# seqsense/pcgol

Measured on AMD Instinct MI355X. Metric: Mpoints/sec ICP iter (corr+reduce) + kNN queries/sec, 1M-pt cloud, higher is better.
Workload: dtype f32

## Files before the change

pcgol_amd/csrc/icp.hip:

```cpp
#include <string.h>

#include <array>
#include <chrono>
#include <condition_variable>
#include <mutex>
#include <string>
#include <thread>

#include <vector>

#include "knn_grid.h"
#include "knn_xwalk.h"
#include "icp_step_plan.h"
#include "strict_terms.h"
#include "gicp_terms.h"

namespace pcgx {

constexpr int kIcpBlock = kKnnBlock;

__device__ __forceinline__ double wave_sum_f64(double v) {
#pragma unroll
  for (int o = 32; o > 0; o >>= 1) v += __shfl_down(v, o);
  return v;
}

__device__ __forceinline__ void accumulate_terms(double *acc, float x0, float y0, float z0, const float4 &bp,
                                                 const IcpKernelParams &kp) {
  const float x1 = bp.x, y1 = bp.y, z1 = bp.z;
  const float w = eval_weight_fn(kp.weight_fn, kp.weight_a, bp.w);
  acc[S_VALUE] += (double)(w * bp.w);
  acc[S_G0 + 0] += (double)(w * (x0 - x1));
  acc[S_G0 + 1] += (double)(w * (y0 - y1));
  acc[S_G0 + 2] += (double)(w * (z0 - z1));
// ... 639 lines not shown
  uint32_t *d_dropped = nullptr;
  int gicp_grid = 1;
  int n_sums() const { return plane ? (int)P_COUNT : (int)S_COUNT; }
  int grid = 1;
  IcpKernelParams kp;
  int32_t max_iteration = 20;
};

static pcgx_status settle(pcgx_icp_session *s, hipStream_t st);
static int icp_knob(const char *name, int def, int lo, int hi);

static IcpKernelParams make_kernel_params(const pcgx_icp_params *p) {
  IcpKernelParams kp;
  memset(&kp, 0, sizeof kp);
  kp.max_dist_sq = p->max_dist * p->max_dist;
  kp.min_dist_sq = p->min_dist_sq;
  kp.min_pairs = p->min_pairs == 0 ? 6 : p->min_pairs;
  kp.upd = resolve_updater(p->weight, p->threshold, p->max_iteration);
  kp.gn = resolve_gauss_newton(p->threshold, 0.0f, p->max_iteration);
  kp.weight_fn = p->weight_fn;
  kp.weight_a = p->weight_fn_param;
  return kp;
}

static int icp_grid(int64_t nt, const TreeView &tv) {
  int64_t blocks = (nt + kIcpBlock - 1) / kIcpBlock;
  int64_t cap = (int64_t)ctx().num_cu * walk_blocks_per_cu(tv) * walk_oversubscribe();
  if (blocks > cap) blocks = cap;
  if (blocks >= 8) blocks &= ~(int64_t)7;
  if (blocks < 1) blocks = 1;
  return (int)blocks;
}

__global__ void icp_reset_kernel(IcpState *__restrict__ state) {
  if (threadIdx.x != 0 || blockIdx.x != 0) return;
  IcpState h;
  memset(&h, 0, sizeof h);
  const Mat4 id = mat4_translate(0.0f, 0.0f, 0.0f);
  for (int i = 0; i < 16; i++) h.trans[i] = id.m[i];
  *state = h;
}

static pcgx_status general_prepare(pcgx_icp_session *s, hipStream_t st) {
  if (s->general_ready) return PCGX_OK;
  const size_t n1 = (size_t)(s->nt ? s->nt : 1);
  PCGX_HIP_TRY(hipMemsetAsync(s->d_match, 0xFF, n1 * sizeof(float4), st));
  PCGX_HIP_TRY(hipMemsetAsync(s->d_match_cert, 0, n1 * sizeof(float), st));
  PCGX_HIP_TRY(hipMemsetAsync(s->d_first_leaf, 0, n1 * sizeof(uint32_t), st));
  PCGX_HIP_TRY(hipMemsetAsync(s->d_walk_count, 0, (size_t)s->grid * sizeof(uint32_t), st));
  s->general_ready = true;
  return PCGX_OK;
}

static pcgx_status reset_state(pcgx_icp_session *s, hipStream_t st) {
  hipLaunchKernelGGL(icp_reset_kernel, dim3(1), dim3(64), 0, st, s->d_state);
  PCGX_HIP_TRY(hipGetLastError());
  s->host_iter = 0;
  if (s->spec_pending) {
    s->spec_pending = false;
    if (s->d_walk_count) PCGX_HIP_TRY(hipMemsetAsync(s->d_walk_count, 0, (size_t)s->grid * sizeof(uint32_t), st));
    PCGX_TRY(strict_reset(s->strict_buf, st));
  }
  if (s->shard_failed || s->steps_sharded > 0) {
    PCGX_TRY(strict_reset(s->strict_buf, st));
    s->shard_failed = false;
    s->steps_sharded = 0;
  }
  return PCGX_OK;
}

extern "C" pcgx_status pcgx_icp_session_reset(pcgx_icp_session *s, void *stream) {
  PCGX_API_LOCK();
  if (!s) return fail(PCGX_E_INVALID, "pcgx_icp_session_reset: NULL session");
  s->touch(pick_stream(stream));
  return reset_state(s, pick_stream(stream));
}

extern "C" pcgx_status pcgx_icp_session_set_pose(pcgx_icp_session *s, const float trans16[16],
                                                 int32_t iter, void *stream) {
  PCGX_API_LOCK();
  if (!s || !trans16 || iter < 0) return fail(PCGX_E_INVALID, "pcgx_icp_session_set_pose: bad argument");
  hipStream_t st = pick_stream(stream);
  s->touch(st);
  PCGX_TRY(settle(s, st));
  IcpState h;
  memset(&h, 0, sizeof h);
  memcpy(h.trans, trans16, sizeof h.trans);
  h.iter = iter;
  s->host_iter = 0;
  PCGX_HIP_TRY(hipMemcpyAsync(s->d_state, &h, sizeof h, hipMemcpyHostToDevice, st));
  PCGX_HIP_TRY(hipStreamSynchronize(st));
  return PCGX_OK;
}

extern "C" pcgx_status pcgx_icp_session_read_sums(pcgx_icp_session *s, double sums10[10], void *stream) {
// ... 1136 lines not shown
```

pcgol_amd/csrc/pcgx_internal.h:

```cpp
#pragma once
#include <hip/hip_runtime.h>
#include <stdint.h>
#include <stdio.h>
#include <stdlib.h>

#include <atomic>
#include <memory>
#include <mutex>
#include <string>
#include <utility>
#include <vector>

#include "../../include/pcgx.h"
#include "pcgx_math.h"

namespace pcgx {

template <class T>
struct DefaultInitAlloc : std::allocator<T> {
  template <class U>
  struct rebind {
    using other = DefaultInitAlloc<U>;
  };
  template <class U>
// ... 220 lines not shown
  UpdaterParams upd;
  GaussNewtonParams gn;
  int32_t weight_fn;
  float weight_a;
};


#if defined(__HIPCC__)
constexpr unsigned int kTicketGroups = 32u, kTicketStride = 32u;
static_assert((1u + kTicketGroups) * kTicketStride * 4u <= kTicketBytes, "the context's ticket words");
__device__ __forceinline__ bool last_workgroup_ticket(unsigned int *tickets) {
  const unsigned int g = blockIdx.x & (kTicketGroups - 1u), groups = min(gridDim.x, kTicketGroups);
  const unsigned int members = (gridDim.x - g + kTicketGroups - 1u) / kTicketGroups;
  unsigned int *mine = tickets + kTicketStride * (1u + g);
  if (atomicAdd(mine, 1u) != members - 1u) return false;
  __hip_atomic_store(mine, 0u, __ATOMIC_RELAXED, __HIP_MEMORY_SCOPE_AGENT);
  if (atomicAdd(tickets, 1u) != groups - 1u) return false;
  __hip_atomic_store(tickets, 0u, __ATOMIC_RELAXED, __HIP_MEMORY_SCOPE_AGENT);
  return true;
}

__device__ __forceinline__ uint32_t wave_incl_scan_u32(uint32_t v) {
#define PCGX_DPP_ADD(CTRL, MASK) v += (uint32_t)__builtin_amdgcn_update_dpp(0, (int)v, CTRL, MASK, 0xf, (MASK) == 0xf)
  PCGX_DPP_ADD(0x111, 0xf);
  PCGX_DPP_ADD(0x112, 0xf);
  PCGX_DPP_ADD(0x114, 0xf);
  PCGX_DPP_ADD(0x118, 0xf);
  PCGX_DPP_ADD(0x142, 0xa);
  PCGX_DPP_ADD(0x143, 0xc);
#undef PCGX_DPP_ADD
  return v;
}
__device__ __forceinline__ void icp_update_step(IcpState *__restrict__ state, const double *__restrict__ sums10,
                                                const IcpKernelParams &kp) {
  state->num_iteration += 1;
  const int64_t npairs = (int64_t)sums10[S_PAIRS];
  if (npairs < (int64_t)kp.min_pairs) {
    state->ev.num_pairs = npairs;
    state->status = PCGX_E_NOT_ENOUGH_PAIRS;
    state->done = 1;
    return;
  }
  Evaluated ev;
  finish_evaluate(sums10, ev);
  state->ev = ev;
  Mat4 t;
  for (int i = 0; i < 16; i++) t.m[i] = state->trans[i];
  int32_t it = state->iter;
  const bool converged = gradient_descent_update(kp.upd, it, ev.gradient, t);
  for (int i = 0; i < 16; i++) state->trans[i] = t.m[i];
  state->iter = it;
  if (converged) state->done = 1;
}

#endif

struct StrictBuffers;
struct StrictWork;
struct CertifiedTerms;
pcgx_status strict_create(int64_t nt, const float *tx, const float *ty, const float *tz, const uint32_t *pos_of,
                          StrictBuffers **out, hipStream_t st);
void strict_destroy(StrictBuffers *b);
const StrictWork *strict_work(StrictBuffers *b, const IcpKernelParams &kp);
pcgx_status strict_enqueue(StrictBuffers *b, const float4 *match, const uint32_t *pos_of, IcpState *state,
                           double *sums10, const IcpKernelParams &kp, bool fuse_update, bool have_tile_sums, bool first_iter,
                           hipStream_t st, const struct CertifiedTerms *certify = nullptr);
pcgx_status strict_read_debug(StrictBuffers *b, unsigned long long out[64], hipStream_t st);
pcgx_status strict_check_enqueue(const float *d_xyz, int64_t nt, int64_t nt_pad, const float4 *match, const uint32_t *pos_of,
                                 IcpState *state, const IcpKernelParams &kp, float *d_terms, unsigned long long *d_valid,
                                 double *d_sums, bool fuse_update, hipStream_t st);
pcgx_status strict_enqueue_sharded(StrictBuffers *b, const float4 *match, const uint32_t *pos_of, IcpState *state,
                                   double *sums10, const IcpKernelParams &kp, pcgx_comm *c, int rank, int world,
                                   bool local_failed, hipStream_t st);
struct RingView {
  unsigned long long *words = nullptr;
  unsigned long long *host = nullptr;
  unsigned long long *const *tab = nullptr;
  unsigned long long *mine = nullptr;
  int32_t words_per_rank = 0, rank = 0, world = 1;
  uint32_t epoch = 0;
  int32_t kind = 0;
  long long guess_ticks = 0;
};
pcgx_status strict_enqueue_ring(StrictBuffers *b, const float4 *match, const uint32_t *pos_of, IcpState *state, double *sums10,
                                const IcpKernelParams &kp, const RingView &ring, bool local_failed, bool first_iter, hipStream_t st);
void ring_abort_from_host(const RingView &ring, uint32_t reason);
pcgx_status strict_reset(StrictBuffers *b, hipStream_t st);
bool small_fit_eligible(const TreeView &tv, int64_t nt, bool many_ties);
size_t small_fit_sync_bytes();
size_t small_fit_terms_bytes(int64_t nt);
int small_fit_max_iters();
bool small_fit_wants_order(int64_t nt);
pcgx_status small_fit_prepare(const float *d_target_aos, int64_t nt, const float box_lo[3], const float box_hi[3], int32_t *d_perm, float *d_xyz,
                               uint32_t *d_pos_of, IcpState *state, void *terms, void *sync, hipStream_t st);
pcgx_status small_fit_enqueue(const TreeView &tv, const float *tx, const float *ty, const float *tz, int64_t nt, IcpState *state,
                              const IcpKernelParams &kp, void *terms, unsigned long long *valid, double *sums10, void *sync,
                              uint32_t launch_no, int iters, const int32_t *perm, hipStream_t st, volatile uint32_t *mailbox = nullptr,
                              uint32_t mailbox_seq = 0u);
bool comm_ring_step(pcgx_comm *c, int32_t step, RingView *out);
void comm_ring_new_fit(pcgx_comm *c);
int comm_ring_kind(pcgx_comm *c);
void comm_attach_local_ring(pcgx_comm *c, unsigned long long *block, int32_t words_per_rank);
}

struct pcgx_kdtree {
  int64_t n = 0;
  int32_t depth = 0;
  float4 *d_nodes = nullptr;
  uint32_t *d_dir = nullptr;
  uint32_t *d_inv = nullptr;
  int32_t dir_bits = 0;
  float dir_lo[3] = {0, 0, 0}, dir_scale[3] = {0, 0, 0};
  float bbox_lo[3] = {0, 0, 0}, bbox_hi[3] = {0, 0, 0};
  bool has_nan = false;
  bool many_ties = false;
  pcgx::RawVector<int32_t> inorder;
  pcgx::RawVector<float> points;
  struct XNode {
    int32_t id, c0, c1, dim;
  };
// ... 35 lines not shown
```

pcgol_amd/csrc/strict.hip:

```cpp
#include <stddef.h>

#include "knn_grid.h"
#include "strict_terms.h"

namespace pcgx {

__device__ __forceinline__ int lane_next(int v, int edge) { return __builtin_amdgcn_update_dpp(edge, v, 0x130, 0xf, 0xf, false); }
__device__ __forceinline__ int lane_prev(int v, int edge) { return __builtin_amdgcn_update_dpp(edge, v, 0x138, 0xf, 0xf, false); }
__device__ __forceinline__ double wave_excl_scan_f64(double v, int lane) {
  double inc = v;
  inc += dpp_f64<0x111, 0xf>(0.0, inc);
  inc += dpp_f64<0x112, 0xf>(0.0, inc);
  inc += dpp_f64<0x114, 0xf>(0.0, inc);
  inc += dpp_f64<0x118, 0xf>(0.0, inc);
  inc += dpp_f64<0x142, 0xa>(0.0, inc);
  inc += dpp_f64<0x143, 0xc>(0.0, inc);
  (void)lane;
  return dpp_f64<0x138, 0xf>(0.0, inc);
}
__device__ __forceinline__ uint32_t wave_all_umin(uint32_t v) {
#define PCGX_DPP_U32(CTRL, MASK) (uint32_t) __builtin_amdgcn_update_dpp(-1, (int)v, CTRL, MASK, 0xf, false)
  v = umin(v, PCGX_DPP_U32(0x111, 0xf));
  v = umin(v, PCGX_DPP_U32(0x112, 0xf));
  v = umin(v, PCGX_DPP_U32(0x114, 0xf));
// ... 260 lines not shown
                                             ChainRange &cr, double &tile_err) {
  g = f2u((float)(base + pre));
  const float e = u2f(plain_chain_q(q, g));
  const double err = ((double)e - (double)u2f(g)) - lsum;
  const double epre = wave_excl_scan_f64(err, lane);
  tile_err = lane_f64(epre, 63) + lane_f64(err, 63);
  const uint32_t g2 = f2u((float)(base + pre + epre));
  const int32_t moved = (int32_t)g2 - (int32_t)g;
  if (__ballot(moved > 2 || moved < -2) != 0ull) g = g2;
  cr = guess_chain_q(q, g);
}
__device__ __forceinline__ void tile_guesses_pair(const LdsQuads &q, double base, double lsum, double pre, int lane, uint32_t &g,
                                                  ChainRange &cr, ChainRange &crb, double &tile_err) {
  g = f2u((float)(base + pre));
  const float e = u2f(plain_chain_q(q, g));
  const double err = ((double)e - (double)u2f(g)) - lsum;
  const double epre = wave_excl_scan_f64(err, lane);
  tile_err = lane_f64(epre, 63) + lane_f64(err, 63);
  const uint32_t g2 = f2u((float)(base + pre + epre));
  const int32_t moved = (int32_t)g2 - (int32_t)g;
  if (__ballot(moved > 2 || moved < -2) != 0ull) g = g2;
  guess_chain_pair_q(q, g, cr, crb);
}

constexpr int kExactTiles = 1;
constexpr uint32_t kPlainMargin = 512u;
constexpr uint32_t kMaybeMargin = 1u << 17;

constexpr int kSumBlock = 512;
constexpr int kSumWaves = kSumBlock / 64;
enum { JOB_CROSSING = 1, JOB_NOWINDOW = 2 };

constexpr long long kExchangeTicks = 200000;
__device__ __forceinline__ void certified_search(const CertifiedTerms &C, const TermSrc &S, const IcpState *state, const StrictWork &W,
                                                 int64_t tile, const uint16_t *list, int nl, float4 *terms ,
                                                 int *np_more) {
  TermSrc S0 = S;
  S0.project = false;
  for (int j = threadIdx.x; j < nl; j += kSumBlock) {
    const int q = list[j];
    const int64_t c = tile * kTile + q;
    float x = W.xyz_caller[3 * c], y = W.xyz_caller[3 * c + 1], z = W.xyz_caller[3 * c + 2];
    float ub = __builtin_inff();
    if (S.project) {
      float px, py, pz;
      mat4_transform(S.m, x, y, z, px, py, pz);
      x = px; y = py; z = pz;
      const float4 pm = C.match_caller[c];
      const float dx = pm.x - x, dy = pm.y - y, dz = pm.z - z;
      const float dm = (dx * dx + dy * dy) + dz * dz;
      if (pm.w >= 0.0f && dm == dm) ub = dm;
    }
    float4 best = make_float4(0.0f, 0.0f, 0.0f, __int_as_float(-1));
    float best_d = C.max_dist_sq;
    GridVerdict v = grid_nearest(C.grid, x, y, z, C.max_dist_sq, ub, best, best_d);
    if (C.test_force_grid_walk && c % C.test_force_grid_walk == 0) v = GRID_WALK;
    if (v == GRID_WALK) {
      if (atomicCAS(&const_cast<IcpState *>(state)->done, 0, 2) == 0) atomicAdd(&W.dbg[47], 1ull << 32);
      continue;
    }
    const bool found = __float_as_int(best.w) >= 0;
    const float cert = (v == GRID_FOUND && found) ? C.grid.cert[__float_as_uint(best.w)] : 0.0f;
    const uint32_t pos = C.pos_of[c];
    C.match[pos] = make_float4(best.x, best.y, best.z, found ? best_d : -1.0f);
    C.match_cert[pos] = cert;
    C.match_caller[c] = make_float4(best.x, best.y, best.z, found ? cert : -1.0f);
    if (found) {
      float t[kStrictRows];
      (void)pair_terms(S0, x, y, z, make_float4(best.x, best.y, best.z, best_d), t);
      const int l = q / kLeaf, vq = (q % kLeaf) / 4, cc = q % 4;
#pragma unroll
      for (int k = 0; k < kStrictRows; k++) reinterpret_cast<float *>(&terms[k * (kTile / 4) + tile_quad(l, vq)])[cc] = t[k];
      atomicAdd(np_more, 1);
    }
  }
}

template <bool kExchange, bool kSharded = false, bool kCertify = false>
__global__ __launch_bounds__(kSumBlock) __attribute__((amdgpu_waves_per_eu(4, 4))) void strict_sum_kernel(
    const float4 *__restrict__ match, const uint32_t *__restrict__ pos_of, const IcpState *__restrict__ state, StrictWork W,
    CertifiedTerms C = CertifiedTerms()) {
  __shared__ float4 s_terms[kStrictRows][kTile / 4];
  __shared__ int s_np[kSumWaves];
  __shared__ double s_tot[16];
  __shared__ uint16_t s_list[kCertify ? kTile : 1];
  __shared__ int s_nlist, s_np_more;
  static_assert(!kSharded || kExchange, "the ring form rides on the exchange");
  static_assert(!kCertify || (kExchange && !kSharded), "the certified terms: one GPU, with the exchange");
  const int done = state->done;
  const int lane = threadIdx.x & 63, wave = threadIdx.x >> 6;
  const int64_t tile = blockIdx.x;
  const int NR = W.nrows;
  const long long t_0 = trace_clock(W);
  long long t_x0 = 0;
  double P0 = (!kExchange && wave < NR) ? tile_prefix(W.tile_sum, W.ntiles, wave, tile, lane) : 0.0;
  {
    const TermSrc S = make_term_src(match, pos_of, state, W);
    const int l = threadIdx.x >> 3, v = threadIdx.x & 7;
    float4 bp[4];
    float tx[4], ty[4], tz[4];
    const int64_t i0 = tile * kTile + (int64_t)l * kLeaf + 4 * v;
    load_quad(S, i0, bp, tx, ty, tz);
    if (kCertify) {
      if (threadIdx.x == 0) s_nlist = s_np_more = 0;
      __syncthreads();
    }
    float t[4][kStrictRows];
    int np = 0;
#pragma unroll
    for (int c = 0; c < 4; c++) {
      if (kCertify) {
        float x = tx[c], y = ty[c], z = tz[c];
        if (S.project) mat4_transform(S.m, tx[c], ty[c], tz[c], x, y, z);
        const float dx = bp[c].x - x, dy = bp[c].y - y, dz = bp[c].z - z;
        const float dm = (dx * dx + dy * dy) + dz * dz;
        bool kept = S.project && bp[c].w >= 0.0f && dm < bp[c].w && dm < C.max_dist_sq;
        if ((C.test_force_walk && (i0 + c) % C.test_force_walk == 0) || (C.test_force_grid_walk && (i0 + c) % C.test_force_grid_walk == 0))
          kept = false;
        if (!kept && i0 + c < W.nt) {
          s_list[atomicAdd(&s_nlist, 1)] = (uint16_t)(l * kLeaf + 4 * v + c);
          bp[c].w = -1.0f;
        }
      }
      np += pair_terms(S, tx[c], ty[c], tz[c], bp[c], t[c]) ? 1 : 0;
    }
#pragma unroll
    for (int k = 0; k < kStrictRows; k++) s_terms[k][tile_quad(l, v)] = make_float4(t[0][k], t[1][k], t[2][k], t[3][k]);
#pragma unroll
    for (int o = 32; o > 0; o >>= 1) np += __shfl_xor(np, o);
    if (lane == 0) s_np[wave] = np;
  }
  __syncthreads();
  if (done) return;
  if (kCertify) {
    const int nl = s_nlist;
    if (nl > 0) {
      certified_search(C, make_term_src(match, pos_of, state, W), state, W, tile, s_list, nl, &s_terms[0][0], &s_np_more);
      __syncthreads();
    }
    if (threadIdx.x == 0) {
      if (tile == 0) atomicAdd(&W.dbg[47], 1ull);
      if (nl > 0) atomicAdd(&W.dbg[59], (unsigned long long)nl);
    }
  }
  if (threadIdx.x == 0) {
    int np = kCertify ? s_np_more : 0;
    for (int w = 0; w < kSumWaves; w++) np += s_np[w];
    W.tile_pairs[tile] = (uint32_t)np;
  }
  static_assert(kStrictRows <= 2 * kSumWaves, "a wave has at most two rows");
  double lsum_kept[2] = {0.0, 0.0}, pre_kept[2] = {0.0, 0.0};
  if (kExchange) {
#pragma unroll
    for (int pass = 0; pass < 2; pass++) {
      const int row = wave + pass * kSumWaves;
      if (row >= NR) break;
      const LdsQuads q{s_terms[row], lane};
      double lsum = 0.0;
#pragma unroll
      for (int v = 0; v < kLeaf / 4; v++) {
        const float4 a = q(v);
        lsum += (double)a.x; lsum += (double)a.y; lsum += (double)a.z; lsum += (double)a.w;
      }
      const double pre = wave_excl_scan_f64(lsum, lane);
      lsum_kept[pass] = lsum;
      pre_kept[pass] = pre;
      if (lane == 63) s_tot[row] = pre + lsum;
    }
    __syncthreads();
    t_x0 = trace_clock(W);
    if (wave == 0) {
      if (lane < NR) {
        const double v = s_tot[lane];
        __hip_atomic_store(&W.tile_pub[(int64_t)lane * W.ntiles_pad + tile], v, __ATOMIC_RELAXED, __HIP_MEMORY_SCOPE_AGENT);
        W.tile_sum[(int64_t)lane * W.ntiles + tile] = v;
      }
      asm volatile("s_waitcnt vmcnt(0)" ::: "memory");
      const int64_t g_mine = tile >> 5, n_groups = (W.ntiles + 31) >> 5;
      if (lane == 0) {
// ... 152 lines not shown
      }
      T.s = par_expand(S, E, key);
      if (lane == 0) W.recs[row * W.ntiles + tile] = T;
      maybe_E = (m_lo < kMaybeMargin || m_hi > 0x7fffffu - kMaybeMargin) ? (int32_t)E : -1;
      if (maybe_E < 0) continue;
    }
    unsigned slot = 0xffffffffu;
    const unsigned shard = (unsigned)((tile + 7 * row) % kAuxShards), per_shard = (unsigned)W.naux / kAuxShards;
    if (lane == 0) {
      const unsigned k = atomicAdd(&W.aux_count[shard * 32], 1u);
      slot = k < per_shard ? shard * per_shard + k : 0xffffffffu;
    }
    slot = (unsigned)rfl((int)slot);
    if (slot == 0xffffffffu) {
      if (maybe_E < 0) {
        T.key = -1;
        T.cons = 0;
        if (lane == 0) W.recs[row * W.ntiles + tile] = T;
      }
      continue;
    }
    if (lane == 0) {
      JobDesc *J = W.jobs + slot;
      J->row = row;
      J->tile = tile;
      J->pad = maybe_E >= 0 ? (1 | (maybe_E << 8)) : 0;
    }
    float4 *dst = W.aux_terms + (size_t)slot * (kTile / 4);
    int lane_here = lane;
    asm volatile("" : "+v"(lane_here));
#pragma unroll
    for (int v = 0; v < kLeaf / 4; v++) dst[v * kLanes + lane_here] = s_terms[row][v * kLanes + lane_here];
  }
  if (threadIdx.x == 0 && (W.selfcheck & 2)) {
    W.stamps[tile * 16 + 0] = (unsigned long long)t_0;
    W.stamps[tile * 16 + 1] = (unsigned long long)t_1;
    W.stamps[tile * 16 + 2] = (unsigned long long)t_x0;
    W.stamps[tile * 16 + 5] = (unsigned long long)trace_clock(W);
  }
}

constexpr int kJobBlock = 256;
constexpr int kJobRoles = 3;
template <bool kRegs>
__device__ __forceinline__ uint32_t resolve_staged(uint32_t s, int kind, int32_t key, const LeafAux &A, int lane,
                                               const float4 *lds, const float *t, int &serial_out, int &tried_out,
                                               int &applied_out);
__global__ __launch_bounds__(kJobBlock) void strict_job_kernel(const IcpState *__restrict__ state, StrictWork W) {
  __shared__ float4 s_t[kTile / 4];
  __shared__ float4 s_lin[kTile / 4];
  __shared__ int32_t s_S[12][kLanes];
  __shared__ uint32_t s_g[kLanes];
  __shared__ int32_t s_lk[kLanes];
  __shared__ int32_t s_hdr[5];
  __shared__ uint32_t s_ctab[4][kCandInner];
  __shared__ int s_cdone, s_pieces;
  const unsigned per_shard = (unsigned)W.naux / kAuxShards;
  const int lane = threadIdx.x & 63, part = threadIdx.x >> 6;
  const int role = (int)(blockIdx.x % kJobRoles);
  const unsigned jb = blockIdx.x / kJobRoles;
  const unsigned shard = jb % kAuxShards, slot = shard * per_shard + jb / kAuxShards;
  const JobDesc *J = W.jobs + slot;
  const float4 *src4 = W.aux_terms + (size_t)slot * (kTile / 4);
  static_assert(kTile / 4 == 2 * kJobBlock, "two quads of the tile per thread");
  const bool early = jb / kAuxShards < 6;
  float4 q0 = make_float4(0.0f, 0.0f, 0.0f, 0.0f), q1 = q0;
  int row = 0, pad = 0;
  int64_t tile = 0;
  if (early) {
    q0 = src4[threadIdx.x];
// ... 544 lines not shown
struct ChainMail {
  int req;
  int ack;
  uint32_t s_in, s_out;
};

template <bool kCheck, bool kSpec = false>
__global__ __launch_bounds__(kChainBlock) void strict_chain_kernel(const float4 *__restrict__ match,
                                                                  const uint32_t *__restrict__ pos_of,
                                                                  IcpState *__restrict__ state, StrictWork W,
                                                                  double *__restrict__ sums10, IcpKernelParams kp,
                                                                  int fuse_update) {
  __shared__ RecArray s_rec;
  __shared__ RecArray s_pre;
  __shared__ RecArray s_suf;
  __shared__ int16_t s_tail[kChainTiles];
  __shared__ int16_t s_head[kChainTiles];
  __shared__ int16_t s_auxlist[kChainTiles];
  __shared__ int16_t s_auxord[kChainTiles];
  __shared__ int32_t s_count[kChainSegs], s_auxcnt[kChainSegs];
  __shared__ uint32_t s_auxmask[kChainSegs][2];
  __shared__ int s_sufok[kChainSegs];
  __shared__ int s_pre_cnt[2];
  __shared__ int s_progress;
  __shared__ ChainMail s_mail[kChainSegs];
  __shared__ uint32_t s_tab[kTabSlots][kCand];
  __shared__ int s_tab_ord[kTabSlots];
  __shared__ float4 s_tile[kTile / 4];
  __shared__ unsigned long long s_np;
  __shared__ int s_np_ok;
  __shared__ uint32_t s_stat[8];
  __shared__ unsigned long long s_wk[8];
  __shared__ unsigned long long s_stat_ticks[2];
  const int done = state->done;
  const int row = (int)(blockIdx.x % (unsigned)W.nrows), my_chunk = (int)(blockIdx.x / (unsigned)W.nrows);
  const int lane = threadIdx.x & 63, wave = rfl((int)(threadIdx.x >> 6));
  const bool walker = wave == kWalker;
  const bool last_chunk = my_chunk == W.nchunks - 1;
  auto term_src = [&]() { return make_term_src(match, pos_of, state, W); };
  uint32_t s = W.start_bits ? (uint32_t)rfl((int)W.start_bits[row]) : f2u(0.0f);
  int ring_rc = 0;
  auto row_start = [&]() -> uint32_t {
    if (!W.ring || W.rank == 0) return W.start_bits ? (uint32_t)rfl((int)W.start_bits[row]) : f2u(0.0f);
    const RingLayout RL{W.world};
    uint32_t v = 0u;
    ring_rc = ring_wait(W, RL.start(row), v, kRingWalkTicks);
    if (ring_rc == 2 && lane == 0) ring_raise_abort(W, 0x100u | (uint32_t)row);
    return (uint32_t)rfl((int)v);
  };
  uint32_t n_run = 0, n_runfail = 0, n_recfail = 0, n_tab_nw = 0, n_tab_cross = 0;
  uint32_t n_mail = 0;
  asm volatile("" : "+v"(n_run), "+v"(n_runfail), "+v"(n_recfail), "+v"(n_tab_nw), "+v"(n_tab_cross), "+v"(n_mail));
  unsigned long long ticks_scan = 0, ticks_walk = 0;
  const long long t_enter = trace_clock(W);
  const unsigned long long c_enter = (W.selfcheck & 2) ? (unsigned long long)__builtin_readcyclecounter() : 0ull;
  {
    const int64_t chunk = (int64_t)my_chunk * kChainTiles;
    const long long t_a = stat_clock(W);
    if (threadIdx.x < kChainSegs) {
      s_sufok[threadIdx.x] = 0;
      s_mail[threadIdx.x].req = 0;
      s_mail[threadIdx.x].ack = 0;
    }
    if (threadIdx.x < kTabSlots) s_tab_ord[threadIdx.x] = 0;
    if (threadIdx.x == 0) {
      s_progress = 0;
      s_pre_cnt[0] = s_pre_cnt[1] = 0;
      s_np_ok = 0;
    }
    if (threadIdx.x < 8) s_wk[threadIdx.x] = 0ull;
    TileRec R;
    R.key = -2;
    R.in = R.out = 0u;
    R.cons = 0;
    R.s = summary_identity();
    bool head = true, tail = true, valid = false;
    {
      const int64_t tile = chunk + threadIdx.x;
      valid = tile < W.ntiles;
      if (valid) R = W.recs[row * W.ntiles + tile];
      if ((W.selfcheck & 2) && last_chunk && walker) {
        const unsigned long long tt = clock_after((uint32_t)R.key);
        if (lane == 0) s_wk[4] = tt;
      }
      rec_put(s_rec, threadIdx.x, R);
      const int32_t key_prev = lane_prev(R.key, R.key), key_next = lane_next(R.key, R.key);
      const int alone = stands_alone(R) ? 1 : 0, alone_prev = lane_prev(alone, 0), alone_next = lane_next(alone, 0);
      head = lane == 0 || R.key < 0 || R.key != key_prev || alone || alone_prev;
      tail = lane == 63 || R.key < 0 || R.key != key_next || alone || alone_next;
      const unsigned long long tails = __ballot(tail && valid);
      if (tail && valid) {
        const unsigned long long below = tails & ((1ull << lane) - 1ull);
        const int idx = wave * 64 + __popcll(below);
        s_tail[idx] = (int16_t)threadIdx.x;
        s_head[idx] = (int16_t)(wave * 64 + (below ? 64 - __builtin_clzll(below) : 0));
      }
      if (lane == 0) s_count[wave] = __popcll(tails);
      const unsigned long long aux = __ballot(valid && (R.cons >> 8) != 0);
      if (lane == 0) {
        s_auxcnt[wave] = __popcll(aux);
        s_auxmask[wave][0] = (uint32_t)aux;
        s_auxmask[wave][1] = (uint32_t)(aux >> 32);
      }
// ... 784 lines not shown
      return;
    }
    if (row == 0 && lane == 0) __hip_atomic_store(&sums10[S_PAIRS], (double)pairs, __ATOMIC_RELAXED, __HIP_MEMORY_SCOPE_AGENT);
  } else if (row == 0 && walker && lane == 0) {
    while (lds_get(&s_np_ok) == 0) __builtin_amdgcn_s_sleep(1);
    if (!W.hop_out) __hip_atomic_store(&sums10[S_PAIRS], (double)s_np, __ATOMIC_RELAXED, __HIP_MEMORY_SCOPE_AGENT);
  }
  if (walker) {
    unsigned ticket = 0u;
    if (lane == 0) {
      const int slot = row == 0 ? S_VALUE : (row <= 6 ? S_G0 + row - 1 : (row == 7 ? S_DIST_RMS : S_WEIGHT));
      if (W.hop_out) W.hop_out[row] = (double)s;
      else __hip_atomic_store(&sums10[slot], (double)u2f(s), __ATOMIC_RELAXED, __HIP_MEMORY_SCOPE_AGENT);
      if (W.hop_out) __threadfence();
      else asm volatile("s_waitcnt vmcnt(0)" ::: "memory");
      ticket = atomicAdd(W.done_rows, 1u);
    }
    ticket = (unsigned)rfl((int)ticket);
    if (ticket == (unsigned)W.nrows - 1u) {
      static_assert(kAuxShards == kLanes, "a shard's counter per lane");
      W.aux_count[lane * 32] = 0u;
      if (W.exchange)
        for (int64_t k = lane, n = (W.ntiles + 31) / 32, m = n + (n + 31) / 32; k < m; k += kLanes) W.tile_arrived[32 * k] = 0u;
      if (lane == 0) *W.done_rows = 0u;
      if (!W.hop_out && lane == 0) {
        double sums[S_COUNT];
        for (int k = 0; k < S_COUNT; k++) sums[k] = __hip_atomic_load(&sums10[k], __ATOMIC_RELAXED, __HIP_MEMORY_SCOPE_AGENT);
        const unsigned long long np = (unsigned long long)sums[S_PAIRS];
        if (W.nrows < kStrictRows) {
          sums[S_WEIGHT] = (double)(np < (1ull << 24) ? np : (1ull << 24));
          sums10[S_WEIGHT] = sums[S_WEIGHT];
        }
        const long long t_u0 = trace_clock(W);
        if (fuse_update) icp_update_step(state, sums, kp);
        if (W.selfcheck & 2) {
          __threadfence();
          W.stamps[kStrictRows * 16 + 14] = (unsigned long long)t_u0;
          W.stamps[kStrictRows * 16 + 15] = (unsigned long long)trace_clock(W);
        }
      }
    }
  }
}

struct StrictBuffers {
  StrictWork w;
  void *block = nullptr;
  double *shard = nullptr;
  int shard_world = 0;
  bool shard_ring = false;
  void *counters = nullptr;
  size_t counters_bytes = 0, arrived_bytes = 0;
};

pcgx_status strict_create(int64_t nt, const float *tx, const float *ty, const float *tz, const uint32_t *pos_of,
                          StrictBuffers **out, hipStream_t st) {
  StrictBuffers *b = new StrictBuffers();
  StrictWork &W = b->w;
  W.nt = nt;
  W.raw_terms = nullptr;
  W.row_base = W.err_base = nullptr;
  W.start_bits = nullptr;
  W.hop_out = nullptr;
  W.first_exact = 1;
  W.ring = nullptr;
  W.ring_words = 0;
  W.ring_tab = nullptr;
// ... 347 lines not shown
    ProfScope prof(PCGX_PROF_STRICT_SUM, st);
    hipLaunchKernelGGL((strict_sum_kernel<true, true>), dim3((unsigned)W.ntiles), dim3(kSumBlock), 0, st, match, pos_of,
                       (const IcpState *)state, W);
  }
  if (ring.world > 1)
    hipLaunchKernelGGL(strict_ring_err_kernel, dim3(kStrictRows + (ring.rank > 0 ? 1 : 0)), dim3(64), 0, st, (const IcpState *)state, W);
  if (ring.rank > 0) {
    W.row_base = W.ring_base;
    W.err_base = W.ring_base + 16;
  }
  {
    ProfScope prof(PCGX_PROF_STRICT_JOB, st);
    if (first_iter && W.naux > 0 && W.ntiles >= kRepairMinTiles && repair_enabled())
      hipLaunchKernelGGL(strict_repair_kernel, dim3((unsigned)(W.nrows * ((W.ntiles + kRepairBlock - 1) / kRepairBlock))), dim3(kRepairBlock), 0,
                         st, match, pos_of, (const IcpState *)state, W);
    if (W.naux > 0)
      hipLaunchKernelGGL(strict_job_kernel, dim3((unsigned)kJobRoles * (unsigned)W.naux), dim3(kJobBlock), 0, st, (const IcpState *)state, W);
  }
  {
    ProfScope prof(PCGX_PROF_STRICT_CHAIN, st);
    launch_chain(W, match, pos_of, state, sums10, kp, 1, true, st);
  }
  PCGX_HIP_TRY(hipGetLastError());
  return PCGX_OK;
}

pcgx_status strict_reset(StrictBuffers *b, hipStream_t st) {
  if (!b) return PCGX_OK;
  PCGX_HIP_TRY(hipMemsetAsync(b->counters, 0, b->counters_bytes, st));
  PCGX_HIP_TRY(hipMemsetAsync(b->w.tile_arrived, 0, b->arrived_bytes, st));
  return PCGX_OK;
}

pcgx_status strict_read_debug(StrictBuffers *b, unsigned long long out[64], hipStream_t st) {
  PCGX_HIP_TRY(hipMemcpyAsync(out, b->w.dbg, 64 * sizeof(unsigned long long), hipMemcpyDeviceToHost, st));
  PCGX_HIP_TRY(hipStreamSynchronize(st));
  if (const char *path = getenv("PCGX_STRICT_TRACE")) {
    std::vector<unsigned long long> h((size_t)b->w.ntiles * 16);
    PCGX_HIP_TRY(hipMemcpy(h.data(), b->w.stamps, h.size() * 8, hipMemcpyDeviceToHost));
    if (FILE *f = fopen(path, "a")) {
      for (int64_t k = 0; k < b->w.ntiles; k++) {
        for (int j = 0; j < 16; j++) fprintf(f, "%llu ", h[(size_t)k * 16 + j]);
        fprintf(f, "\n");
      }
      fprintf(f, "#\n");
      fclose(f);
    }
  }
  if (const char *path = getenv("PCGX_STRICT_KEYS")) {
    std::vector<TileRec> h((size_t)kStrictRows * b->w.ntiles);
    PCGX_HIP_TRY(hipMemcpy(h.data(), b->w.recs, h.size() * sizeof(TileRec), hipMemcpyDeviceToHost));
    if (FILE *f = fopen(path, "a")) {
      for (int r = 0; r < kStrictRows; r++) {
        for (int64_t k = 0; k < b->w.ntiles; k++) fprintf(f, "%d:%d ", h[(size_t)r * b->w.ntiles + k].key, h[(size_t)r * b->w.ntiles + k].cons);
        fprintf(f, "\n");
      }
      fprintf(f, "#\n");
      fclose(f);
    }
  }
  PCGX_HIP_TRY(hipMemsetAsync(b->w.dbg, 0, 64 * sizeof(unsigned long long), st));
  return PCGX_OK;
}

}

// ... 72 lines not shown
```

Baseline: 14890.

## Wave-cooperative certified search, fold reset memsets into kernel, prefetch pose for update

After: 15230 (median of 6 runs). 2.3% higher.

```diff
diff --git a/pcgol_amd/csrc/icp.hip b/pcgol_amd/csrc/icp.hip
--- a/pcgol_amd/csrc/icp.hip
+++ b/pcgol_amd/csrc/icp.hip
@@ -1,5 +1,6 @@
 #include <string.h>
 
+#include <algorithm>
 #include <array>
 #include <chrono>
 #include <condition_variable>
@@ -705,7 +706,14 @@
   return (int)blocks;
 }
 
-__global__ void icp_reset_kernel(IcpState *__restrict__ state) {
+struct IcpResetZero {
+  uint32_t *p[3] = {nullptr, nullptr, nullptr};
+  uint32_t words[3] = {0u, 0u, 0u};
+};
+__global__ void icp_reset_kernel(IcpState *__restrict__ state, IcpResetZero z) {
+#pragma unroll
+  for (int r = 0; r < 3; r++)
+    for (uint32_t i = blockIdx.x * blockDim.x + threadIdx.x; i < z.words[r]; i += gridDim.x * blockDim.x) z.p[r][i] = 0u;
   if (threadIdx.x != 0 || blockIdx.x != 0) return;
   IcpState h;
   memset(&h, 0, sizeof h);
@@ -726,14 +734,27 @@
 }
 
 static pcgx_status reset_state(pcgx_icp_session *s, hipStream_t st) {
-  hipLaunchKernelGGL(icp_reset_kernel, dim3(1), dim3(64), 0, st, s->d_state);
+  IcpResetZero z;
+  size_t zero_words = 0;
+  if (s->spec_pending) {
+    s->spec_pending = false;
+    void *ptr[2];
+    size_t bytes[2];
+    strict_reset_ranges(s->strict_buf, ptr, bytes);
+    if (s->d_walk_count) {
+      z.p[0] = s->d_walk_count;
+      z.words[0] = (uint32_t)s->grid;
+    }
+    for (int r = 0; r < 2; r++) {
+      z.p[1 + r] = (uint32_t *)ptr[r];
+      z.words[1 + r] = (uint32_t)(bytes[r] / sizeof(uint32_t));
+    }
+    for (int r = 0; r < 3; r++) zero_words += z.words[r];
+  }
+  const unsigned blocks = zero_words ? (unsigned)std::min<size_t>((zero_words + 1023) / 1024, 64) : 1u;
+  hipLaunchKernelGGL(icp_reset_kernel, dim3(blocks), dim3(zero_words ? 256 : 64), 0, st, s->d_state, z);
   PCGX_HIP_TRY(hipGetLastError());
   s->host_iter = 0;
-  if (s->spec_pending) {
-    s->spec_pending = false;
-    if (s->d_walk_count) PCGX_HIP_TRY(hipMemsetAsync(s->d_walk_count, 0, (size_t)s->grid * sizeof(uint32_t), st));
-    PCGX_TRY(strict_reset(s->strict_buf, st));
-  }
   if (s->shard_failed || s->steps_sharded > 0) {
     PCGX_TRY(strict_reset(s->strict_buf, st));
     s->shard_failed = false;
diff --git a/pcgol_amd/csrc/pcgx_internal.h b/pcgol_amd/csrc/pcgx_internal.h
--- a/pcgol_amd/csrc/pcgx_internal.h
+++ b/pcgol_amd/csrc/pcgx_internal.h
@@ -276,8 +276,9 @@
   return v;
 }
 __device__ __forceinline__ void icp_update_step(IcpState *__restrict__ state, const double *__restrict__ sums10,
-                                                const IcpKernelParams &kp) {
-  state->num_iteration += 1;
+                                                const IcpKernelParams &kp, const float *pose_in = nullptr,
+                                                const int32_t *count_in = nullptr) {
+  state->num_iteration = (count_in ? count_in[1] : state->num_iteration) + 1;
   const int64_t npairs = (int64_t)sums10[S_PAIRS];
   if (npairs < (int64_t)kp.min_pairs) {
     state->ev.num_pairs = npairs;
@@ -289,8 +290,8 @@
   finish_evaluate(sums10, ev);
   state->ev = ev;
   Mat4 t;
-  for (int i = 0; i < 16; i++) t.m[i] = state->trans[i];
-  int32_t it = state->iter;
+  for (int i = 0; i < 16; i++) t.m[i] = pose_in ? pose_in[i] : state->trans[i];
+  int32_t it = count_in ? count_in[0] : state->iter;
   const bool converged = gradient_descent_update(kp.upd, it, ev.gradient, t);
   for (int i = 0; i < 16; i++) state->trans[i] = t.m[i];
   state->iter = it;
@@ -330,6 +331,7 @@
                                 const IcpKernelParams &kp, const RingView &ring, bool local_failed, bool first_iter, hipStream_t st);
 void ring_abort_from_host(const RingView &ring, uint32_t reason);
 pcgx_status strict_reset(StrictBuffers *b, hipStream_t st);
+void strict_reset_ranges(StrictBuffers *b, void *ptr[2], size_t bytes[2]);
 bool small_fit_eligible(const TreeView &tv, int64_t nt, bool many_ties);
 size_t small_fit_sync_bytes();
 size_t small_fit_terms_bytes(int64_t nt);
diff --git a/pcgol_amd/csrc/strict.hip b/pcgol_amd/csrc/strict.hip
--- a/pcgol_amd/csrc/strict.hip
+++ b/pcgol_amd/csrc/strict.hip
@@ -316,48 +316,113 @@
 enum { JOB_CROSSING = 1, JOB_NOWINDOW = 2 };
 
 constexpr long long kExchangeTicks = 200000;
-__device__ __forceinline__ void certified_search(const CertifiedTerms &C, const TermSrc &S, const IcpState *state, const StrictWork &W,
-                                                 int64_t tile, const uint16_t *list, int nl, float4 *terms ,
-                                                 int *np_more) {
-  TermSrc S0 = S;
-  S0.project = false;
-  for (int j = threadIdx.x; j < nl; j += kSumBlock) {
-    const int q = list[j];
-    const int64_t c = tile * kTile + q;
-    float x = W.xyz_caller[3 * c], y = W.xyz_caller[3 * c + 1], z = W.xyz_caller[3 * c + 2];
-    float ub = __builtin_inff();
-    if (S.project) {
-      float px, py, pz;
-      mat4_transform(S.m, x, y, z, px, py, pz);
-      x = px; y = py; z = pz;
-      const float4 pm = C.match_caller[c];
-      const float dx = pm.x - x, dy = pm.y - y, dz = pm.z - z;
-      const float dm = (dx * dx + dy * dy) + dz * dz;
-      if (pm.w >= 0.0f && dm == dm) ub = dm;
-    }
+__device__ __forceinline__ int nth_set_bit(unsigned long long m, int n) {
+  int pos = 0;
+#pragma unroll
+  for (int w = 32; w > 0; w >>= 1) {
+    const int cnt = __popcll(m & (((1ull << w) - 1ull) << pos));
+    const bool up = n >= cnt;
+    n -= up ? cnt : 0;
+    pos += up ? w : 0;
+  }
+  return pos;
+}
+
+struct CertifiedStore {
+  float4 best;
+  float best_d;
+  uint32_t pos;
+  int32_t q;
+};
+__device__ __forceinline__ void certified_store_flush(const CertifiedTerms &C, int64_t tile, CertifiedStore &D) {
+  if (D.q < 0) return;
+  const bool found = __float_as_int(D.best.w) >= 0;
+  const float cert = (D.q & 0x10000) ? C.grid.cert[__float_as_uint(D.best.w)] : 0.0f;
+  const int64_t c = tile * kTile + (D.q & 0xffff);
+  C.match[D.pos] = make_float4(D.best.x, D.best.y, D.best.z, found ? D.best_d : -1.0f);
+  C.match_cert[D.pos] = cert;
+  C.match_caller[c] = make_float4(D.best.x, D.best.y, D.best.z, found ? cert : -1.0f);
+  D.q = -1;
+}
+
+__device__ __forceinline__ int certified_wave_search(const CertifiedTerms &C, const IcpState *state, const StrictWork &W, int64_t tile,
+                                                      int lane, int wave, const bool (&fail)[4], float (&mx)[4], float (&my)[4],
+                                                      float (&mz)[4], const float (&ub)[4], float4 (&bp)[4], float4 *park,
+                                                      CertifiedStore &D) {
+  constexpr int kStride = kTile / 4;
+  unsigned long long m[4];
+  int base[5];
+  base[0] = 0;
+#pragma unroll
+  for (int c = 0; c < 4; c++) {
+    m[c] = __ballot(fail[c]);
+    base[c + 1] = base[c] + __popcll(m[c]);
+  }
+  const int n = base[4];
+  if (n == 0) return 0;
+#pragma unroll 1
+  for (int r0 = 0; r0 < n; r0 += kLanes) {
+    certified_store_flush(C, tile, D);
+    const bool on = r0 + lane < n;
+    const int k = on ? r0 + lane : r0;
+    const int c = (k >= base[1] ? 1 : 0) + (k >= base[2] ? 1 : 0) + (k >= base[3] ? 1 : 0);
+    const unsigned long long mc = c == 0 ? m[0] : (c == 1 ? m[1] : (c == 2 ? m[2] : m[3]));
+    const int bc = c == 0 ? base[0] : (c == 1 ? base[1] : (c == 2 ? base[2] : base[3]));
+    const int owner = nth_set_bit(mc, k - bc);
+    float x = 0.0f, y = 0.0f, z = 0.0f, u = 0.0f;
+#pragma unroll
+    for (int cc = 0; cc < 4; cc++) {
+      const float gx = __shfl(mx[cc], owner), gy = __shfl(my[cc], owner), gz = __shfl(mz[cc], owner), gu = __shfl(ub[cc], owner);
+      x = c == cc ? gx : x;
+      y = c == cc ? gy : y;
+      z = c == cc ? gz : z;
+      u = c == cc ? gu : u;
+    }
+#pragma unroll
+    for (int cc = 0; cc < 4; cc++) park[cc * kStride] = bp[cc];
+    park[4 * kStride] = make_float4(mx[0], mx[1], mx[2], mx[3]);
+    park[5 * kStride] = make_float4(my[0], my[1], my[2], my[3]);
+    park[6 * kStride] = make_float4(mz[0], mz[1], mz[2], mz[3]);
     float4 best = make_float4(0.0f, 0.0f, 0.0f, __int_as_float(-1));
     float best_d = C.max_dist_sq;
-    GridVerdict v = grid_nearest(C.grid, x, y, z, C.max_dist_sq, ub, best, best_d);
-    if (C.test_force_grid_walk && c % C.test_force_grid_walk == 0) v = GRID_WALK;
-    if (v == GRID_WALK) {
-      if (atomicCAS(&const_cast<IcpState *>(state)->done, 0, 2) == 0) atomicAdd(&W.dbg[47], 1ull << 32);
-      continue;
-    }
-    const bool found = __float_as_int(best.w) >= 0;
-    const float cert = (v == GRID_FOUND && found) ? C.grid.cert[__float_as_uint(best.w)] : 0.0f;
-    const uint32_t pos = C.pos_of[c];
-    C.match[pos] = make_float4(best.x, best.y, best.z, found ? best_d : -1.0f);
-    C.match_cert[pos] = cert;
-    C.match_caller[c] = make_float4(best.x, best.y, best.z, found ? cert : -1.0f);
-    if (found) {
-      float t[kStrictRows];
-      (void)pair_terms(S0, x, y, z, make_float4(best.x, best.y, best.z, best_d), t);
-      const int l = q / kLeaf, vq = (q % kLeaf) / 4, cc = q % 4;
-#pragma unroll
-      for (int k = 0; k < kStrictRows; k++) reinterpret_cast<float *>(&terms[k * (kTile / 4) + tile_quad(l, vq)])[cc] = t[k];
-      atomicAdd(np_more, 1);
-    }
-  }
+    float w_new = -1.0f;
+    __builtin_amdgcn_s_setprio(3);
+    if (on) {
+      const int q = 4 * (wave * kLanes + owner) + c;
+      const int64_t cg = tile * kTile + q;
+      const uint32_t pos = C.pos_of[cg];
+      GridVerdict v = grid_nearest(C.grid, x, y, z, C.max_dist_sq, u, best, best_d);
+      if (C.test_force_grid_walk && cg % C.test_force_grid_walk == 0) v = GRID_WALK;
+      if (v == GRID_WALK) {
+        if (atomicCAS(&const_cast<IcpState *>(state)->done, 0, 2) == 0) atomicAdd(&W.dbg[47], 1ull << 32);
+      } else {
+        const bool found = __float_as_int(best.w) >= 0;
+        w_new = found ? best_d : -1.0f;
+        D.best = best;
+        D.best_d = best_d;
+        D.pos = pos;
+        D.q = q | ((v == GRID_FOUND && found) ? 0x10000 : 0);
+      }
+    }
+    __builtin_amdgcn_s_setprio(0);
+    float4 *back = park;
+    asm volatile("" : "+v"(back));
+#pragma unroll
+    for (int cc = 0; cc < 4; cc++) bp[cc] = back[cc * kStride];
+    const float4 px = back[4 * kStride], py = back[5 * kStride], pz = back[6 * kStride];
+    mx[0] = px.x; mx[1] = px.y; mx[2] = px.z; mx[3] = px.w;
+    my[0] = py.x; my[1] = py.y; my[2] = py.z; my[3] = py.w;
+    mz[0] = pz.x; mz[1] = pz.y; mz[2] = pz.z; mz[3] = pz.w;
+#pragma unroll
+    for (int cc = 0; cc < 4; cc++) {
+      const int src = base[cc] + __popcll(m[cc] & ((1ull << lane) - 1ull)) - r0;
+      const bool got = ((m[cc] >> lane) & 1ull) && src >= 0 && src < kLanes;
+      const int sl = got ? src : lane;
+      const float rx = __shfl(best.x, sl), ry = __shfl(best.y, sl), rz = __shfl(best.z, sl), rw = __shfl(w_new, sl);
+      if (got) bp[cc] = make_float4(rx, ry, rz, rw);
+    }
+  }
+  return n;
 }
 
 template <bool kExchange, bool kSharded = false, bool kCertify = false>
@@ -366,9 +431,8 @@
     CertifiedTerms C = CertifiedTerms()) {
   __shared__ float4 s_terms[kStrictRows][kTile / 4];
   __shared__ int s_np[kSumWaves];
+  __shared__ int s_ns[kCertify ? kSumWaves : 1];
   __shared__ double s_tot[16];
-  __shared__ uint16_t s_list[kCertify ? kTile : 1];
-  __shared__ int s_nlist, s_np_more;
   static_assert(!kSharded || kExchange, "the ring form rides on the exchange");
   static_assert(!kCertify || (kExchange && !kSharded), "the certified terms: one GPU, with the exchange");
   const int done = state->done;
@@ -377,6 +441,8 @@
   const int NR = W.nrows;
   const long long t_0 = trace_clock(W);
   long long t_x0 = 0;
+  CertifiedStore held;
+  held.q = -1;
   double P0 = (!kExchange && wave < NR) ? tile_prefix(W.tile_sum, W.ntiles, wave, tile, lane) : 0.0;
   {
     const TermSrc S = make_term_src(match, pos_of, state, W);
@@ -385,15 +451,13 @@
     float tx[4], ty[4], tz[4];
     const int64_t i0 = tile * kTile + (int64_t)l * kLeaf + 4 * v;
     load_quad(S, i0, bp, tx, ty, tz);
-    if (kCertify) {
-      if (threadIdx.x == 0) s_nlist = s_np_more = 0;
-      __syncthreads();
-    }
     float t[4][kStrictRows];
     int np = 0;
-#pragma unroll
-    for (int c = 0; c < 4; c++) {
-      if (kCertify) {
+    if (kCertify) {
+      bool fail[4];
+      float ub[4];
+#pragma unroll
+      for (int c = 0; c < 4; c++) {
         float x = tx[c], y = ty[c], z = tz[c];
         if (S.project) mat4_transform(S.m, tx[c], ty[c], tz[c], x, y, z);
         const float dx = bp[c].x - x, dy = bp[c].y - y, dz = bp[c].z - z;
@@ -401,12 +465,21 @@
         bool kept = S.project && bp[c].w >= 0.0f && dm < bp[c].w && dm < C.max_dist_sq;
         if ((C.test_force_walk && (i0 + c) % C.test_force_walk == 0) || (C.test_force_grid_walk && (i0 + c) % C.test_force_grid_walk == 0))
           kept = false;
-        if (!kept && i0 + c < W.nt) {
-          s_list[atomicAdd(&s_nlist, 1)] = (uint16_t)(l * kLeaf + 4 * v + c);
-          bp[c].w = -1.0f;
-        }
-      }
-      np += pair_terms(S, tx[c], ty[c], tz[c], bp[c], t[c]) ? 1 : 0;
+        fail[c] = !kept && i0 + c < W.nt;
+        ub[c] = (S.project && bp[c].w >= 0.0f && dm == dm) ? dm : __builtin_inff();
+        if (fail[c]) bp[c].w = -1.0f;
+        tx[c] = x; ty[c] = y; tz[c] = z;
+      }
+      int ns = 0;
+      if (!done) ns = certified_wave_search(C, state, W, tile, lane, wave, fail, tx, ty, tz, ub, bp, &s_terms[0][tile_quad(l, v)], held);
+      if (lane == 0) s_ns[wave] = ns;
+      TermSrc S0 = S;
+      S0.project = false;
+#pragma unroll
+      for (int c = 0; c < 4; c++) np += pair_terms(S0, tx[c], ty[c], tz[c], bp[c], t[c]) ? 1 : 0;
+    } else {
+#pragma unroll
+      for (int c = 0; c < 4; c++) np += pair_terms(S, tx[c], ty[c], tz[c], bp[c], t[c]) ? 1 : 0;
     }
 #pragma unroll
     for (int k = 0; k < kStrictRows; k++) s_terms[k][tile_quad(l, v)] = make_float4(t[0][k], t[1][k], t[2][k], t[3][k]);
@@ -415,20 +488,10 @@
     if (lane == 0) s_np[wave] = np;
   }
   __syncthreads();
+  const long long t_p1 = trace_clock(W);
   if (done) return;
-  if (kCertify) {
-    const int nl = s_nlist;
-    if (nl > 0) {
-      certified_search(C, make_term_src(match, pos_of, state, W), state, W, tile, s_list, nl, &s_terms[0][0], &s_np_more);
-      __syncthreads();
-    }
-    if (threadIdx.x == 0) {
-      if (tile == 0) atomicAdd(&W.dbg[47], 1ull);
-      if (nl > 0) atomicAdd(&W.dbg[59], (unsigned long long)nl);
-    }
-  }
   if (threadIdx.x == 0) {
-    int np = kCertify ? s_np_more : 0;
+    int np = 0;
     for (int w = 0; w < kSumWaves; w++) np += s_np[w];
     W.tile_pairs[tile] = (uint32_t)np;
   }
@@ -647,10 +710,20 @@
 #pragma unroll
     for (int v = 0; v < kLeaf / 4; v++) dst[v * kLanes + lane_here] = s_terms[row][v * kLanes + lane_here];
   }
+  if (kCertify) {
+    certified_store_flush(C, tile, held);
+    if (threadIdx.x == 0) {
+      if (tile == 0) atomicAdd(&W.dbg[47], 1ull);
+      int ns = 0;
+      for (int w = 0; w < kSumWaves; w++) ns += s_ns[w];
+      if (ns > 0) atomicAdd(&W.dbg[59], (unsigned long long)ns);
+    }
+  }
   if (threadIdx.x == 0 && (W.selfcheck & 2)) {
     W.stamps[tile * 16 + 0] = (unsigned long long)t_0;
     W.stamps[tile * 16 + 1] = (unsigned long long)t_1;
     W.stamps[tile * 16 + 2] = (unsigned long long)t_x0;
+    W.stamps[tile * 16 + 3] = (unsigned long long)t_p1;
     W.stamps[tile * 16 + 5] = (unsigned long long)trace_clock(W);
   }
 }
@@ -1261,6 +1334,8 @@
   __shared__ uint32_t s_stat[8];
   __shared__ unsigned long long s_wk[8];
   __shared__ unsigned long long s_stat_ticks[2];
+  __shared__ float s_pose[16];
+  __shared__ int32_t s_pose_n[2];
   const int done = state->done;
   const int row = (int)(blockIdx.x % (unsigned)W.nrows), my_chunk = (int)(blockIdx.x / (unsigned)W.nrows);
   const int lane = threadIdx.x & 63, wave = rfl((int)(threadIdx.x >> 6));
@@ -1298,6 +1373,11 @@
       s_np_ok = 0;
     }
     if (threadIdx.x < 8) s_wk[threadIdx.x] = 0ull;
+    static_assert(kWalker != 0, "wave 0 fetches the loop state: it must not be the walker");
+    if (fuse_update && threadIdx.x < 18) {
+      if (threadIdx.x < 16) s_pose[threadIdx.x] = state->trans[threadIdx.x];
+      else s_pose_n[threadIdx.x - 16] = threadIdx.x == 16 ? state->iter : state->num_iteration;
+    }
     TileRec R;
     R.key = -2;
     R.in = R.out = 0u;
@@ -2148,7 +2228,7 @@
           sums10[S_WEIGHT] = sums[S_WEIGHT];
         }
         const long long t_u0 = trace_clock(W);
-        if (fuse_update) icp_update_step(state, sums, kp);
+        if (fuse_update) icp_update_step(state, sums, kp, s_pose, s_pose_n);
         if (W.selfcheck & 2) {
           __threadfence();
           W.stamps[kStrictRows * 16 + 14] = (unsigned long long)t_u0;
@@ -2562,6 +2642,13 @@
   return PCGX_OK;
 }
 
+void strict_reset_ranges(StrictBuffers *b, void *ptr[2], size_t bytes[2]) {
+  ptr[0] = b ? b->counters : nullptr;
+  bytes[0] = b ? b->counters_bytes : 0;
+  ptr[1] = b ? (void *)b->w.tile_arrived : nullptr;
+  bytes[1] = b ? b->arrived_bytes : 0;
+}
+
 pcgx_status strict_read_debug(StrictBuffers *b, unsigned long long out[64], hipStream_t st) {
   PCGX_HIP_TRY(hipMemcpyAsync(out, b->w.dbg, 64 * sizeof(unsigned long long), hipMemcpyDeviceToHost, st));
   PCGX_HIP_TRY(hipStreamSynchronize(st));
```
